# samxuxiang/BrepGen

Measured on AMD Instinct MI355X. Metric: denoising-steps/sec (whole node), DeepCAD face-LDM, batch=512, higher is better.
Workload: dtype bf16

## Files before the change

brepgen_amd/_lib.py:

```python
import ctypes as C
import os

_HERE = os.path.dirname(os.path.abspath(__file__))
LIB_PATH = os.path.join(_HERE, "libbrepgen_hip.so")

BG_F32, BG_F16, BG_BF16 = 0, 1, 2
BG_ACT_NONE, BG_ACT_RELU = 0, 1
BG_SURFPOS, BG_SURFZ, BG_EDGEPOS, BG_EDGEZ = 0, 1, 2, 3
BG_MAX_LAYERS, BG_MAX_EMBEDS = 12, 5
BG_ATTN_BWD_AUTO, BG_ATTN_BWD_GENERAL, BG_ATTN_BWD_SHORT = 0, 1, 2

vp, fp, i64p, u8p = C.c_void_p, C.c_void_p, C.c_void_p, C.c_void_p


class MlpWeights(C.Structure):
    _fields_ = [("w0", vp), ("b0", fp), ("ln_g", fp), ("ln_b", fp), ("w3", vp), ("b3", fp),
                ("k_in", C.c_int), ("n_out", C.c_int), ("n_out_pad", C.c_int), ("w0_dtype", C.c_int),
                ("w0_mfma", fp), ("w0_colsum", fp)]


class LayerWeights(C.Structure):
    _fields_ = [("ln1_g", fp), ("ln1_b", fp), ("ln2_g", fp), ("ln2_b", fp),
                ("w_qkv", vp), ("b_qkv", fp), ("w_o", vp), ("b_o", fp),
                ("w_1", vp), ("b_1", fp), ("w_2", vp), ("b_2", fp),
# ... 120 lines not shown
                               fp, fp, fp, C.c_float, C.c_float, C.c_float, C.c_float, C.c_float, fp,
                               C.c_size_t, vp]),
    "bg_groupnorm_stats": (C.c_int, [fp, fp, C.c_int, C.c_int, C.c_int, C.c_int, C.c_float, vp]),
    "bg_im2col": (C.c_int, [fp, vp] + [C.c_int] * 13 + [fp, fp, fp, C.c_int, C.c_int, fp, vp]),
    "bg_downsample1d_cubic": (C.c_int, [fp, fp, C.c_int, C.c_int, C.c_int, vp]),
    "bg_upsample1d_cubic": (C.c_int, [fp, fp, C.c_int, C.c_int, C.c_int, vp]),
    "bg_small_attn": (C.c_int, [fp, C.c_int, vp, C.c_int, C.c_int, C.c_int, C.c_int, C.c_int, C.c_float, vp]),
    "bg_dedup_surfaces": (C.c_int, [fp, C.c_float, fp, u8p, C.c_int, C.c_int, vp]),
    "bg_dedup_edges": (C.c_int, [fp, u8p, C.c_float, u8p, C.c_int, C.c_int, C.c_int, vp]),
    "bg_profile_begin": (C.c_int, [C.c_int]),
    "bg_profile_end": (C.c_int, [C.POINTER(ProfileRow), C.c_int]),
    "bg_tune_set": (C.c_int, [C.c_int, C.c_int]),
    "bg_allgather": (C.c_int, [vp, vp, C.c_size_t, vp, vp]),
    "bg_slot_packing_applies": (C.c_int, [C.c_int] * 6),
    "bg_gemm_p256_rows": (C.c_int, [C.c_int, C.c_int, C.c_int, C.c_int]),
    "bg_add_noise": (C.c_int, [fp, fp, fp, fp, fp, C.c_int, C.c_size_t, vp]),
    "bg_chamfer_offset_fit": (C.c_int, [fp, fp, vp, C.c_int, C.c_int, C.c_int] + [C.c_double] * 5 + [fp, fp, fp, vp]),
    "bg_philox_randn": (C.c_int, [fp, C.c_longlong, C.c_int, C.c_ulonglong, C.c_uint, C.c_longlong, C.c_int, vp]),
    "bg_masked_mse": (C.c_int, [fp, fp, u8p, C.c_longlong, C.c_int, C.c_int, C.c_int, vp, fp, vp]),
    "bg_chamfer_pairwise": (C.c_int, [fp, C.c_int, C.c_int, fp, C.c_int, C.c_int, fp, vp]),
    "bg_occupancy_counts": (C.c_int, [fp, C.c_int, C.c_int, fp, C.c_int, vp, vp, vp]),
    "bg_mesh_sample": (C.c_int, [fp, vp, C.c_int, C.c_int, C.c_ulonglong, C.c_uint, C.c_longlong, fp, fp, fp, vp, fp, vp]),
    "bg_vae_posterior": (C.c_int, [fp, fp, C.c_longlong, C.c_int, C.c_int, C.c_ulonglong, C.c_uint, C.c_longlong, fp, fp, fp, vp]),
    "bg_cad_filter": (C.c_int, [C.POINTER(CadStore), C.c_int, C.c_int, C.c_float, C.c_double, u8p, vp]),
    "bg_batch_plan": (C.c_int, [C.POINTER(CadStore), vp, C.c_int, C.c_int, C.c_int, C.c_int, C.c_int, C.c_ulonglong, C.c_uint,
                                C.POINTER(BatchDraws), vp, vp, vp, fp, vp]),
    "bg_batch_gather": (C.c_int, [C.POINTER(CadStore), C.c_int, C.c_int, C.c_int, C.c_int, C.c_float, vp, vp, vp, fp,
                                  C.POINTER(BatchOut), vp]),
    "bg_points_rotate_normalize": (C.c_int, [fp, C.c_longlong, C.c_int, C.c_int, C.c_ulonglong, C.c_uint, C.c_longlong, fp, vp, fp, vp]),
    "bg_points_sha256": (C.c_int, [fp, C.c_longlong, C.c_int, C.c_int, u8p, vp]),
# ... 110 lines not shown
```

brepgen_amd/csrc/bg_common.h:

```cpp
#pragma once
#include <hip/hip_runtime.h>
#include <stdint.h>
#include <stddef.h>
#include <type_traits>
#include "../../include/brepgen_hip.h"

namespace bg {

void set_error(const char* fmt, ...);
int launch_status(const char* what);

#define BG_REQUIRE(cond, code, ...)            \
    do {                                       \
        if (!(cond)) {                         \
            ::bg::set_error(__VA_ARGS__);      \
            return (code);                     \
        }                                      \
    } while (0)

inline bool aligned(const void* p, size_t bytes) { return ((uintptr_t)p & (bytes - 1)) == 0; }
template <typename F> inline void with_bools(bool a, bool b, F&& f) {
    if (a && b) f(std::true_type{}, std::true_type{});
    else if (a) f(std::true_type{}, std::false_type{});
    else if (b) f(std::false_type{}, std::true_type{});
// ... 1 lines not shown
}

enum ProfKernel { PK_GEMM_BF16_128 = 0,   PK_GEMM_BF16_64, PK_GEMM_F32, PK_ATTN_BF16, PK_ATTN_F32, PK_LAYERNORM,
                  PK_DDPM_STEP, PK_PNDM_STEP, PK_MISC, PK_EMBED, PK_GEMM_P256, PK_GEMM_SPLIT, PK_GEMM_P256_SPLIT, PK_QKV_ATTN, PK_OUT_TAIL, PK_FFN_FUSED, PK_COUNT };
extern bool g_prof_on;
void prof_pre(hipStream_t s);
void prof_post(int kernel, double flops, double bytes, hipStream_t s);
struct ProfScope {
    int k; double f, b; hipStream_t s;
    ProfScope(int kernel, double flops, double bytes, hipStream_t st) : k(kernel), f(flops), b(bytes), s(st) {
        if (g_prof_on) prof_pre(s);
    }
    ~ProfScope() { if (g_prof_on) prof_post(k, f, b, s); }
};

enum TuneKey { TUNE_GEMM_STAGGER = 8, TUNE_P256_MODE = 10, TUNE_SPLIT_PIPE = 12, TUNE_QKV_ATTN = 13, TUNE_QKV_WALK = 14, TUNE_SMALL_TILES = 15, TUNE_FFN_FUSED = 16, TUNE_DEBUG_PTR_LO = 17, TUNE_DEBUG_PTR_HI = 18, TUNE_VAE_GN1_FUSED = 19, TUNE_ATTN_WALK = 20, TUNE_COUNT = 21 };
extern int g_tune[TUNE_COUNT];

typedef __attribute__((ext_vector_type(8))) __bf16 bf16x8;
typedef __attribute__((ext_vector_type(4))) __bf16 bf16x4;
typedef __attribute__((ext_vector_type(4))) _Float16 half4_t;
typedef __attribute__((ext_vector_type(8))) _Float16 half8_t;
typedef __attribute__((ext_vector_type(16))) float f32x16;
typedef __attribute__((ext_vector_type(4))) float f32x4;
typedef __attribute__((ext_vector_type(8))) float f32x8;

constexpr int WAVE = 64;

__device__ __forceinline__ float wave_sum(float v) {
#pragma unroll
    for (int o = 32; o > 0; o >>= 1) v += __shfl_xor(v, o, 64);
// ... 55 lines not shown
    int gemv_ok = 0;
    const int* m_dev = nullptr;
    const int* row_map = nullptr;
    int map_add = 0, map_add2 = 0, map_out = 0;
    double rows_hint = 0.0;
    double rows_plan = 0.0;
    int cv_C = 0, cv_H = 0, cv_W = 0, cv_kh = 1, cv_kw = 1, cv_up = 0;
    int cv_wo_log2 = 0, cv_ho_log2 = 0, cv_spt_log2 = 0;
    const void* cv_zero = nullptr;
    int hybrid = 0;
    const int* rule_table = nullptr;
    const int* rows256_dev = nullptr;
    int rows256_host = 0;
    int p256_stagger = 0;
    int concurrent = 0;
};

inline GemmArgs linear(const void* a, int lda, const void* w, const float* bias, void* out, int ldc, int M, int N, int N_pad, int K,
                       int out_dtype, int act = BG_ACT_NONE) {
    return GemmArgs{a, lda, w, bias, out, ldc, M, N, N_pad, K, out_dtype, act, nullptr, 0, 1};
}
inline void add_rows(GemmArgs& g, const float* add, int ld, int div) { g.add = add; g.ld_add = ld; g.add_div = add ? div : 1; }
inline void add2_rows(GemmArgs& g, const float* add2, int ld, int div) { g.add2 = add2; g.ld_add2 = ld; g.add2_div = add2 ? div : 1; }
inline void split_out(GemmArgs& g, void* lo, float* stats) { g.out_lo = lo; g.stats_out = stats; }
inline void split_residual_in(GemmArgs& g, const void* hi, const void* lo, int ld) { g.res_hi = hi; g.res_lo = lo; g.ld_res = ld; }
inline void ln_fold_in(GemmArgs& g, const float* stats, const float* colsum) { g.stats_in = stats; g.colsum = colsum; }
inline void map_rows(GemmArgs& g, const int* row_map, bool add, bool add2, bool out) {
    g.row_map = row_map; g.map_add = add; g.map_add2 = add2; g.map_out = out;
}

// ... 17 lines not shown
    if (rem == 0 || rem >= 200) return panels << 8;
    return (R * q) << 8;
}
__host__ __device__ inline int p256_rows(int rows, int nt_n256, bool split = false, bool all_or_nothing = false) {
    const int panels = (rows + 255) >> 8, T = panels * nt_n256;
    if (all_or_nothing) {
        if (split) return p256_split_rows(panels, nt_n256, true);
        return (T >= 300 || (T >= 200 && T <= 256)) ? panels << 8 : 0;
    }
    if (split) {
        return p256_split_rows(panels, nt_n256, false);
    }
    const int R = T >> 8, rem = T - (R << 8);
    if (rem == 0 || rem >= P256_TAIL_MIN) return panels << 8;
    return ((R << 8) / nt_n256) << 8;
}

template <bool F16> __device__ __forceinline__ void unpack4_16(uint2 u, float (&f)[4]) {
    if (F16) {
        union { uint2 u; half4_t h; } c; c.u = u;
        f[0] = (float)c.h[0]; f[1] = (float)c.h[1]; f[2] = (float)c.h[2]; f[3] = (float)c.h[3];
    } else {
        f[0] = __uint_as_float(u.x << 16); f[1] = __uint_as_float(u.x & 0xffff0000u);
        f[2] = __uint_as_float(u.y << 16); f[3] = __uint_as_float(u.y & 0xffff0000u);
    }
}
template <bool F16> __device__ __forceinline__ void split4_16(const float (&v)[4], uint2& hi, uint2& lo) {
    hi = pack4_16(v[0], v[1], v[2], v[3], F16 ? BG_F16 : BG_BF16);
    float h[4];
    unpack4_16<F16>(hi, h);
// ... 37 lines not shown
                 int silu, hipStream_t s, const int* m_dev = nullptr, double rows_hint = 0.0);
int layernorm768_split(const void* hi, const void* lo, const float* g, const float* b, void* y, int y_dtype, int M,
                       float eps, hipStream_t s, const int* m_dev = nullptr, double rows_hint = 0.0);
bool embed_ln_silu_supported(int k);
bool gn1_norm_act_supported(int P, int C);
int gn1_norm_act(const float* x, void* out, int out_dtype, int S, int P, int C, const float* gamma, const float* beta, float eps,
                 int act, const float* add, hipStream_t s);
int embed_ln_silu(const float* x, int lda, int rows, int k, const float* w0p, const float* b0, const float* g,
                  const float* b, void* out, int out_dtype, float eps, hipStream_t s, const int* m_dev = nullptr,
                  const int* src_row = nullptr, double rows_hint = 0.0);
int attention(const void* qkv, const uint8_t* key_pad, void* out, int B, int N, int dtype, hipStream_t s,
              const int* offsets = nullptr, double pairs_hint = 0.0, double rows_hint = 0.0);
bool qkv_attn_eligible(int B, int N, int dtype, const void* stats_in, const void* colsum, const void* bias);
bool qkv_attn_worthwhile(int B, int N);
int qkv_attention(const void* x_hi, const void* w_qkv, const float* bias, const float* colsum, const float* stats_in, void* out,
                  const uint8_t* key_pad, int B, int N, int dtype, float ln_eps, hipStream_t s);

int qkv_attention_paired(const void* x_hi, const void* w_qkv, const float* bias, const float* colsum, const float* stats_in, void* out,
                         void* qkv_dbg, const int* m_dev, const int* slot_desc, int slot_bound, int m_stats, int dtype, float ln_eps,
                         hipStream_t s, double rows_hint, double pairs_hint);
int compact_rows_paired(const uint8_t* mask, int B, int n_mask, int* offsets, int* src_row, int* slot_desc, int* slot_a, int* counts,
                        hipStream_t s, int* rule = nullptr);
int compact_rows(const uint8_t* mask, int B, int n_mask, int rep, int* offsets, int* src_row, hipStream_t s, int* rule = nullptr);
int sincos_embed(const int64_t* t, int n, float* out, hipStream_t s);
int cond_vector(const float* temb, int nt, const float* class_embed, const int64_t* label, float* c, int B,
                hipStream_t s);
int cond_vector_table(const float* table, int table_rows, const int64_t* timesteps, int nt, const float* class_embed,
                      const int64_t* label, float* c, int B, hipStream_t s);
bool ln_silu_out_supported(int n_out, int n_out_pad);
int ln_silu_out(const void* t0, const float* gam, const float* bet, const void* w3, const float* b3, float* out, int n_out, int n_out_pad,
                int M, int dtype, float eps, hipStream_t s, const int* m_dev = nullptr, const int* row_map = nullptr, double rows_hint = 0.0);
// ... 16 lines not shown
```

brepgen_amd/csrc/denoiser.hip:

```cpp
#include "bg_common.h"
#include <mutex>

namespace bg {

__global__ void expand_mask_kernel(const uint8_t* __restrict__ in, uint8_t* __restrict__ out, size_t n, int E) {
    for (size_t i = blockIdx.x * (size_t)blockDim.x + threadIdx.x; i < n; i += (size_t)gridDim.x * blockDim.x)
        out[i] = in[i / E];
}

static inline size_t align_up(size_t v) { return (v + 255) & ~(size_t)255; }

struct Workspace {
    size_t off_x, off_h, off_r, off_small, off_f, off_mask, off_stats, off_rows, off_slots, total;
    int M, F;
    int Mrow;
};

static inline bool slot_packing_applies(int net, int B, int S, int E, int dtype) {
    return net == BG_SURFZ && E == 1 && S <= 64 && dtype != BG_F32 && B <= 8192;
}

static Workspace plan(int net, int B, int S, int E, int dtype) {
    Workspace w{};
    const size_t es = (dtype == BG_F32) ? 4 : 2;
// ... 26 lines not shown
    float* X;
    void* H;
    void* R;
    bool fold = false;
    void* XH = nullptr;
    void* XL = nullptr;
    float* stats = nullptr;
    const int* m_dev = nullptr;
    const int* src_row = nullptr;
    const int* offsets = nullptr;
    const int* rule = nullptr;
    const int* slot_desc = nullptr;
    double rows_hint = 0.0, pairs_hint = 0.0;
    double rows_plan = 0.0;
    int concurrent = 0;
    const bg_denoiser_inputs* in = nullptr;
    int net = 0, B = 0, N = 1, E = 1, M = 0;
    bool varlen = false;
    bool paired = false;
    bool fused_qkv = false;
    const uint8_t* key_pad = nullptr;
    float* cvec = nullptr;
};

static void token_rows(const Ctx& c, GemmArgs& g, bool launch_plan = true) {
    g.m_dev = c.m_dev; g.rows_hint = c.rows_hint;
    if (launch_plan) { g.rule_table = c.rule; g.rows_plan = c.rows_plan; g.concurrent = c.concurrent; }
}

struct Addend { const float* rows = nullptr; int ld = 0; int div = 1; };
enum EmbedOpt : unsigned { TO_STREAM = 1, TOK = 2, GATHER = 4, MAP_ADD = 8, MAP_ADD2 = 16, SCATTER = 32 };

static int embed_mlp(Ctx& c, const bg_mlp_weights& m, const void* x, int lda, int rows, float* out, int ldc, Addend add = {},
                     Addend add2 = {}, unsigned opt = 0) {
    int rc;
    const bool vl = (opt & TOK) && c.m_dev != nullptr;
    if (m.w0_mfma && m.w0_dtype == BG_F32 && embed_ln_silu_supported(m.k_in)) {
        rc = embed_ln_silu(reinterpret_cast<const float*>(x), lda, rows, m.k_in, m.w0_mfma, m.b0, m.ln_g, m.ln_b, c.H,
                           c.dtype, 1e-5f, c.s, vl ? c.m_dev : nullptr, (vl && (opt & GATHER)) ? c.src_row : nullptr, vl ? c.rows_hint : 0.0);
        if (rc) return rc;
    } else {
        BG_REQUIRE(!(vl && (opt & GATHER)), BG_E_ARG, "bg_denoiser_fwd: variable-length execution needs the fused input embeds (w0_mfma)");
// ... 40 lines not shown
    if ((rc = gemm(f1, c.dtype, c.s))) return rc;
    GemmArgs f2 = linear(c.R, 1024, L.w_2, L.b_2, c.X, 768, M, 768, 768, 1024, BG_F32);
    add_rows(f2, c.X, 768, 1);
    token_rows(c, f2);
    return gemm(f2, c.dtype, c.s);
}

static int encoder_layer_folded(const Ctx& c, const bg_layer_weights& L) {
    int rc;
    const int M = c.M;
    if (c.paired) {
        if ((rc = qkv_attention_paired(c.XH, L.w_qkv, L.b_qkv, L.qkv_colsum, c.stats, c.H, nullptr, c.m_dev, c.slot_desc,
                                       c.B < (M + 63) / 64 ? c.B : (M + 63) / 64, M, c.dtype,
                                       1e-5f, c.s, c.rows_hint, c.pairs_hint))) return rc;
    } else if (c.fused_qkv) {
        if ((rc = qkv_attention(c.XH, L.w_qkv, L.b_qkv, L.qkv_colsum, c.stats, c.H, c.key_pad, c.B, c.N, c.dtype, 1e-5f, c.s))) return rc;
    } else {
        GemmArgs qkv = linear(c.XH, 768, L.w_qkv, L.b_qkv, c.R, 2304, M, 2304, 2304, 768, c.dtype);
        ln_fold_in(qkv, c.stats, L.qkv_colsum);
        token_rows(c, qkv);
        if ((rc = gemm(qkv, c.dtype, c.s))) return rc;
        if ((rc = attention(c.R, c.key_pad, c.H, c.B, c.N, c.dtype, c.s, c.offsets, c.pairs_hint, c.rows_hint))) return rc;
    }
    GemmArgs op = linear(c.H, 768, L.w_o, L.b_o, c.XH, 768, M, 768, 768, 768, c.dtype);
    split_out(op, c.XL, c.stats);
    split_residual_in(op, c.XH, c.XL, 768);
    token_rows(c, op);
    if ((rc = gemm(op, c.dtype, c.s))) return rc;
    if (L.w_1f && L.w_2f && g_tune[TUNE_FFN_FUSED] != 1) {
        FfnArgs ff{c.XH, c.XL, c.stats, L.w_1f, L.b_1, L.w1_colsum, L.w_2f, L.b_2, M, M, c.m_dev, 1e-5f};
        BG_REQUIRE(ffn_fused_eligible(ff, c.dtype), BG_E_ARG, "bg_denoiser_fwd: w_1f / w_2f given, but the fused FFN launch does not apply");
// ... 160 lines not shown
                   "bg_denoiser_fwd: fc_out carries the folded final LayerNorm (w0_colsum): needs the 16-bit LayerNorm-fold layers and n_out <= 48");
        GemmArgs g0 = linear(c.XH, 768, mo.w0, mo.b0, c.H, 768, M, 768, 768, 768, c.dtype);
        ln_fold_in(g0, c.stats, mo.w0_colsum);
        token_rows(c, g0);
        if ((rc = gemm(g0, c.dtype, c.s))) return rc;
        return ln_silu_out(c.H, mo.ln_g, mo.ln_b, mo.w3, mo.b3, eps_out, mo.n_out, mo.n_out_pad, M, c.dtype, 1e-5f, c.s, c.m_dev,
                           c.varlen ? c.src_row : nullptr, c.rows_hint);
    }
    if (c.fold) rc = layernorm768_split(c.XH, c.XL, c.w->lnf_g, c.w->lnf_b, c.H, c.dtype, M, 1e-5f, c.s, c.m_dev, c.rows_hint);
    else rc = layernorm768(c.X, c.w->lnf_g, c.w->lnf_b, c.H, c.dtype, M, 1e-5f, 0, c.s, c.m_dev, c.rows_hint);
    if (rc) return rc;
    return embed_mlp(c, mo, c.H, 768, M, eps_out, mo.n_out, {}, {}, TOK | SCATTER);
}

static int run(const bg_denoiser_weights* w, const bg_denoiser_inputs* in, float* eps_out, void* workspace,
               size_t ws_bytes, hipStream_t s, bool concurrent = false) {
    int rc;
    if ((rc = check_args(w, in, eps_out, workspace))) return rc;
    Ctx c;
    c.s = s;
    c.concurrent = concurrent ? 1 : 0;
    if ((rc = bind_workspace(c, w, in, workspace, ws_bytes))) return rc;
    if (c.varlen && (rc = setup_varlen(c, eps_out))) return rc;
    if ((rc = cond_vectors(c))) return rc;
    if ((rc = token_embeds(c))) return rc;
    if ((rc = encoder_layers(c))) return rc;
    return output_tail(c, eps_out);
}

}

namespace bg {
constexpr int MAX_SPLIT = 4;
static inline void split_range(int B, int n, int k, int& lo, int& hi) {
    const int base = B / n, rem = B % n;
    lo = k * base + (k < rem ? k : rem);
    hi = lo + base + (k < rem ? 1 : 0);
}
static size_t plan_total_split(int net, int B, int S, int E, int dtype, int n) {
    size_t t = 0;
    for (int k = 0; k < n; ++k) {
        int lo, hi;
        split_range(B, n, k, lo, hi);
        if (hi > lo) t += align_up(plan(net, hi - lo, S, E, dtype).total);
    }
    return t;
}
struct SplitState {
    hipStream_t aux[MAX_SPLIT - 1];
    hipEvent_t fork, join[MAX_SPLIT - 1];
    bool tried = false, ok = false;
};
constexpr int MAX_SPLIT_DEVICES = 64;
// ... 18 lines not shown
extern "C" int bg_slot_packing_applies(int net, int B, int S, int E, int dtype, int fold) {
    if (net < BG_EDGEPOS) E = 1;
    return (bg::slot_packing_applies(net, B, S, E, dtype) && fold != 0 && bg::g_tune[bg::TUNE_QKV_ATTN] != 1) ? 1 : 0;
}

extern "C" size_t bg_workspace_bytes(int net, int B, int S, int E, int dtype) {
    if (B <= 0 || S <= 0) return 0;
    if (net < BG_EDGEPOS) E = 1;
    if (E <= 0) return 0;
    size_t t = bg::plan(net, B, S, E, dtype).total;
    for (int n = 2; n <= bg::MAX_SPLIT; ++n) {
        const size_t ts = bg::plan_total_split(net, B, S, E, dtype, n);
        t = ts > t ? ts : t;
    }
    return t;
}

extern "C" int bg_denoiser_fwd(const bg_denoiser_weights* w, const bg_denoiser_inputs* in, float* eps_out,
                               void* workspace, size_t workspace_bytes, bg_stream_t stream) {
    using namespace bg;
    BG_REQUIRE(w && in, BG_E_ARG, "bg_denoiser_fwd: null descriptor");
    hipStream_t s = (hipStream_t)stream;
    BG_REQUIRE(in->n_split >= 0, BG_E_ARG, "bg_denoiser_fwd: n_split must be >= 0 (got %d)", in->n_split);
    const int ns = in->n_split > MAX_SPLIT ? MAX_SPLIT : in->n_split;
    if (ns < 2 || in->B < ns) return run(w, in, eps_out, workspace, workspace_bytes, s);

    const int net = w->net;
    BG_REQUIRE(net >= BG_SURFPOS && net <= BG_EDGEZ, BG_E_ARG, "bg_denoiser_fwd: bad net id %d", net);
    BG_REQUIRE(in->B > 0 && in->S > 0 && eps_out && workspace, BG_E_ARG, "bg_denoiser_fwd: null pointer / empty shape");
    const int S = in->S, E = (net >= BG_EDGEPOS) ? in->E : 1;
// ... 20 lines not shown
        sub.n_split = 1;
        sub.x = in->x + (size_t)lo * tok * kInCols[net];
        if (in->surf_pos) sub.surf_pos = in->surf_pos + (size_t)lo * S * 6;
        if (in->surf_z) sub.surf_z = in->surf_z + (size_t)lo * S * 48;
        if (in->edge_pos) sub.edge_pos = in->edge_pos + (size_t)lo * tok * 6;
        if (in->mask) sub.mask = in->mask + (size_t)lo * mask_per_sample;
        if (in->n_timesteps == in->B) { sub.timesteps = in->timesteps + lo; sub.n_timesteps = sub.B; }
        if (in->class_label) sub.class_label = in->class_label + lo;
        if (in->cond_cache) sub.cond_cache = in->cond_cache + (size_t)lo * S * 768;
        sub.rows_hint = in->rows_hint * sub.B / in->B;
        sub.pairs_hint = in->pairs_hint * sub.B / in->B;
        sub.rows_plan[0] = in->rows_plan[k];
        const size_t bytes = align_up(plan(net, sub.B, S, E, w->dtype).total);
        hipStream_t sk = k == 0 ? s : g_split.aux[k - 1];
        if (k > 0 && (he = hipStreamWaitEvent(sk, g_split.fork, 0)) != hipSuccess) { rc = (int)he; break; }
        rc = run(w, &sub, eps_out + (size_t)lo * tok * w->fc_out.n_out, wsp, bytes, sk, true);
        if (rc) break;
        wsp += bytes;
    }
    for (int k = 1; k < ns; ++k) {
        if (hipEventRecord(g_split.join[k - 1], g_split.aux[k - 1]) == hipSuccess)
            (void)hipStreamWaitEvent(s, g_split.join[k - 1], 0);
    }
    return rc;
}

extern "C" size_t bg_embed_mlp_scratch_bytes(int rows, int dtype) {
    if (rows <= 0) return 0;
    const size_t es = (dtype == BG_F32) ? 4 : 2;
    return bg::align_up((size_t)rows * 768 * es) + bg::align_up((size_t)rows * 768 * 4);
}
// ... 45 lines not shown
```

brepgen_amd/csrc/gemm_16bit.hip:

```cpp
#include "gemm16.h"

namespace bg {

template <bool F16, int BM, int BN, int WM, int WN, int STAGES>
__global__ __launch_bounds__(WM * WN * 64) void gemm16_kernel(GemmArgs g) {
    using E = Elem<F16>;
    using T = typename E::T;
    using V8 = typename E::V8;
    using V4 = typename E::V4;
    constexpr int NW = WM * WN;
    constexpr int TM = BM / WM / 32, TN = BN / WN / 32;
    constexpr int STAGE_BYTES = (BM + BN) * 128;
    constexpr int EH = TM > 2 ? 2 : TM;
    constexpr int EPI_BYTES = NW * EH * 32 * (BN / WN) * 4;
    constexpr int LDS_BYTES = (STAGES * STAGE_BYTES > EPI_BYTES) ? STAGES * STAGE_BYTES : EPI_BYTES;
    static_assert(LDS_BYTES <= 160 * 1024, "LDS budget");
    static_assert((BM / 8) % NW == 0 && (BN / 8) % NW == 0, "DMA pieces must divide evenly over the waves");
    __shared__ __attribute__((aligned(16))) unsigned char lds[LDS_BYTES];

    const T* __restrict__ A = reinterpret_cast<const T*>(g.a);
    const T* __restrict__ W = reinterpret_cast<const T*>(g.w);
    const int lane = threadIdx.x & 63;
    const int wave = __builtin_amdgcn_readfirstlane(threadIdx.x >> 6);
    const int wm = wave / WN, wn = wave % WN;
// ... 667 lines not shown
        return BG_E_SHAPE;
    }
    GemmArgs gt = g;
    gt.hybrid = 0;
    if (g_tune[TUNE_P256_MODE] != 2 && p256_eligible(g)) {
        const bool split = g.out_lo != nullptr;
        const int hmode = g.concurrent ? 2 : 1;
        auto p256 = [&](GemmArgs h, double rows) {
            double fl, by;
            gemm_cost(g, rows, fl, by);
            ProfScope prof(split ? PK_GEMM_P256_SPLIT : PK_GEMM_P256, fl, by, s);
            if (split) h.p256_stagger = split_stagger(g);
            return launch_p256<F16>(h, s);
        };
        if (g_tune[TUNE_P256_MODE] == 1) return p256(g, rows_all);
        const bool plan = g.m_dev != nullptr && g.rows_plan > 0;
        const int rows_est = plan ? (int)fmin((double)g.M, g.rows_plan + 0.5)
                                  : ((g.m_dev != nullptr && g.rows_hint > 0) ? (int)fmin((double)g.M, g.rows_hint + 0.5) : g.M);
        const int rows_hi = p256_rows(rows_est, g.N_pad / 256, split, hmode == 2);
        if (plan && rows_hi >= rows_est) return p256(g, rows_all);
        const int ridx = p256_rule_index(g.N_pad / 256, split, hmode == 2);
        const bool can_tail = persistent_ok && (!g.stats_in || g.K == FOLD_PARTS * G_BK) &&
                              (g.m_dev == nullptr || (g.rule_table != nullptr && ridx >= 0));
        if (rows_hi > 0 && can_tail) {
            gt.hybrid = hmode;
            if (g.m_dev) gt.rows256_dev = g.rule_table + ridx;
            else gt.rows256_host = p256_rows(g.M, g.N_pad / 256, split, hmode == 2);
            const double rows_p = fmin((double)p256_rows((int)rows_all, g.N_pad / 256, split, hmode == 2), rows_all);
            rows_tail = rows_all - rows_p;
            const int rc = p256(gt, rows_p);
// ... 70 lines not shown
```

brepgen_amd/csrc/gemm_split.hip:

```cpp
#include "gemm16.h"

namespace bg {

constexpr int SP_STAGE = 32768, SP_RING = 2 * SP_STAGE, SP_PATCH = 4096;
typedef __attribute__((ext_vector_type(4))) unsigned sp_u32x4;

template <bool F16>
__global__ __launch_bounds__(256, 2) void gemm16_split_pipe_kernel(GemmArgs g, int m_panels) {
    using E = Elem<F16>;
    using T = typename E::T;
    using V8 = typename E::V8;
    __shared__ __attribute__((aligned(16))) unsigned char lds[SP_RING + 4 * SP_PATCH];

    const int lane = threadIdx.x & 63;
    const int wave = __builtin_amdgcn_readfirstlane(threadIdx.x >> 6);
    const int wm = wave >> 1, wn = wave & 1;
    const int l31 = lane & 31, hq = lane >> 5, k8 = lane & 7, r8 = lane >> 3;
    const int Mv = g.m_dev ? *g.m_dev : g.M;
    if (g.m_dev) m_panels = (Mv + 127) >> 7;
    const PanelWalk128 walk(g, m_panels, g.N_pad >> 7, blockIdx.x, gridDim.x);
    const int w_local = walk.w_local, cnt = walk.cnt;

    const unsigned char* Ab = reinterpret_cast<const unsigned char*>(g.a);
    const unsigned char* Wb = reinterpret_cast<const unsigned char*>(g.w);
// ... 213 lines not shown
}

bool split_pipe_eligible(const GemmArgs& g) {
    if (!(g.out_lo && g.res_hi && g.res_lo && g.stats_out && g.bias) || g.stats_in || g.add || g.add2 || g.row_map || g.act != BG_ACT_NONE ||
        g.cv_C > 0 || g.out_dtype == BG_F32)
        return false;
    if (g.N != g.N_pad || g.N_pad % 128 != 0 || g.K % (4 * G_BK) != 0 || g.K < 12 * G_BK || g.ldc % 8 != 0 || g.ld_res % 8 != 0)
        return false;
    const long long nt = (long long)((g.M + 127) / 128) * (g.N_pad / 128);
    return nt >= 64 && (size_t)127 * g.lda * 2 + 128 < 0xffffffffull && (size_t)127 * g.K * 2 + 128 < 0xffffffffull;
}

template <bool F16>
int launch_split_pipe(const GemmArgs& g, hipStream_t s) {
    const int m128 = (g.M + 127) / 128, nt = m128 * (g.N_pad / 128);
    const int grid = nt < 512 ? (nt & ~7) : 512;
    hipLaunchKernelGGL((gemm16_split_pipe_kernel<F16>), dim3(grid), dim3(256), 0, s, g, m128);
    return launch_status("gemm16_split_pipe");
}
template int launch_split_pipe<false>(const GemmArgs&, hipStream_t);
template int launch_split_pipe<true>(const GemmArgs&, hipStream_t);

}
```

brepgen_amd/csrc/qkv_attn.hip:

```cpp
#include "gemm16.h"
#include <math.h>

namespace bg {

constexpr int QA_BUF = 57344, QA_AHALF = 16384, QA_WOFF = 32768, QA_RING = 2 * QA_BUF;
constexpr int QA_LDS = 163840;
constexpr int QA_AUX = QA_RING, QA_BIAS = QA_LDS - QA_AUX - 2048, QA_CSUM = QA_BIAS + 1024;
constexpr int QA_QIMG = QA_BUF, QA_KIMG = QA_QIMG + 32768, QA_VIMG = QA_KIMG + 32768;

constexpr int QA_MB = QA_AUX + QA_BIAS - 1024;
static_assert(QA_VIMG + 32768 <= QA_MB && QA_VIMG + 32768 <= QA_AUX + QA_BIAS, "the V image ends below the key bias / bias / column sums");

struct QkvAttnArgs {
    const void* a;
    const void* w;
    const float* bias;
    const float* colsum;
    const float* stats_in;
    void* out;
    void* dbg;
    const uint8_t* key_pad;
    int B, N, M;
    float ln_eps;
    const int* m_dev = nullptr;
// ... 417 lines not shown
           (((size_t)stats_in) & 15) == 0 && (size_t)B * N * BG_D_MODEL * 2 < 0xffffffffull;
}

bool qkv_attn_worthwhile(int B, int N) {
    const int spt = N <= 32 ? 8 : 4;
    const int tiles = (B + spt - 1) / spt * BG_N_HEAD;
    return tiles <= 256 || tiles >= 352;
}

static int qkv_attn_pinned_walk(int tiles, int grid) {
    const int t = g_tune[TUNE_QKV_WALK];
    if (t == 1 || (grid & 7) != 0) return 0;
    return (t == 2 || tiles >= 512) ? 1 : 0;
}

int qkv_attention_launch(const QkvAttnArgs& g, int dtype, hipStream_t s) {
    const int S = g.N <= 32 ? 32 : 64, spt = 256 / S;
    const int tiles = (g.B + spt - 1) / spt * BG_N_HEAD;
    if (tiles <= 0) return 0;
    const double rows = (double)g.B * g.N;
    ProfScope prof(PK_QKV_ATTN, 2.0 * rows * BG_D_MODEL * 3 * BG_D_MODEL + 4.0 * BG_N_HEAD * (double)g.B * g.N * g.N * BG_D_HEAD,
                   rows * (2.0 * BG_D_MODEL * 2 + FOLD_PARTS * 8.0) + 2.0 * 3 * BG_D_MODEL * BG_D_MODEL + 2 * 4.0 * 3 * BG_D_MODEL, s);
    const int grid = tiles < 256 ? tiles : 256;
    const bool f16 = dtype == BG_F16;
    QkvAttnArgs ge = g;
    ge.pin = qkv_attn_pinned_walk(tiles, grid);
#define QA_LAUNCH(F, SS, MK, D) hipLaunchKernelGGL((qkv_attn_kernel<F, SS, MK, D>), dim3(grid), dim3(512), 0, s, ge)
#define QA_PICK(MK, D)                                                                                     \
    do {                                                                                                   \
        if (S == 64) { if (f16) QA_LAUNCH(true, 64, MK, D); else QA_LAUNCH(false, 64, MK, D); }           \
        else { if (f16) QA_LAUNCH(true, 32, MK, D); else QA_LAUNCH(false, 32, MK, D); }                   \
    } while (0)
    if (g.dbg) {
        if (g.key_pad) QA_PICK(true, true); else QA_PICK(false, true);
    } else {
        if (g.key_pad) QA_PICK(true, false); else QA_PICK(false, false);
    }
#undef QA_PICK
// ... 14 lines not shown
    const double pairs = pairs_hint > 0 ? pairs_hint : 64.0 * rows;
    ProfScope prof(PK_QKV_ATTN, 2.0 * rows * BG_D_MODEL * 3 * BG_D_MODEL + 4.0 * BG_N_HEAD * pairs * BG_D_HEAD,
                   rows * (2.0 * BG_D_MODEL * 2 + FOLD_PARTS * 8.0) + 2.0 * 3 * BG_D_MODEL * BG_D_MODEL + 2 * 4.0 * 3 * BG_D_MODEL, s);
    const int grid = tiles < 256 ? tiles : 256;
    if (dtype == BG_F16) {
        if (qkv_dbg) hipLaunchKernelGGL((qkv_attn_kernel<true, 64, false, true, true>), dim3(grid), dim3(512), 0, s, g);
        else hipLaunchKernelGGL((qkv_attn_kernel<true, 64, false, false, true>), dim3(grid), dim3(512), 0, s, g);
    } else {
        if (qkv_dbg) hipLaunchKernelGGL((qkv_attn_kernel<false, 64, false, true, true>), dim3(grid), dim3(512), 0, s, g);
        else hipLaunchKernelGGL((qkv_attn_kernel<false, 64, false, false, true>), dim3(grid), dim3(512), 0, s, g);
    }
    return launch_status("qkv_attn_paired");
}

int qkv_attention(const void* x_hi, const void* w_qkv, const float* bias, const float* colsum, const float* stats_in, void* out,
                  const uint8_t* key_pad, int B, int N, int dtype, float ln_eps, hipStream_t s) {
    const QkvAttnArgs g{x_hi, w_qkv, bias, colsum, stats_in, out, nullptr, key_pad, B, N, B * N, ln_eps};
    return qkv_attention_launch(g, dtype, s);
}

}

extern "C" int bg_qkv_attn_fwd(const void* x_hi, const void* w_qkv, const float* bias, const float* colsum, const float* stats_in,
                               const uint8_t* key_pad, void* out, void* qkv_dbg, int B, int N, int dtype, float ln_eps,
                               bg_stream_t stream) {
    BG_REQUIRE(x_hi && w_qkv && out && B >= 0 && N >= 0, BG_E_ARG, "bg_qkv_attn_fwd: null pointer or negative size");
    BG_REQUIRE(bg::qkv_attn_eligible(B, N, dtype, stats_in, colsum, bias), BG_E_SHAPE,
               "bg_qkv_attn_fwd: needs 16-bit operands, an even N in [2, 64], LayerNorm-fold statistics / column sums / bias (16-byte aligned)");
    BG_REQUIRE(((uintptr_t)x_hi & 15) == 0 && ((uintptr_t)w_qkv & 15) == 0 && ((uintptr_t)out & 15) == 0 &&
               ((uintptr_t)bias & 15) == 0 && ((uintptr_t)colsum & 15) == 0, BG_E_ALIGN, "bg_qkv_attn_fwd: 16-byte alignment");
    bg::QkvAttnArgs g{x_hi, w_qkv, bias, colsum, stats_in, out, qkv_dbg, key_pad, B, N, B * N, ln_eps};
    return bg::qkv_attention_launch(g, dtype, (hipStream_t)stream);
}
// ... 15 lines not shown
```

brepgen_amd/csrc/runtime.hip:

```cpp
#include "bg_common.h"
#include <stdarg.h>
#include <stdio.h>

namespace bg {

static thread_local char g_err[512] = "";

void set_error(const char* fmt, ...) {
    va_list ap;
    va_start(ap, fmt);
    vsnprintf(g_err, sizeof(g_err), fmt, ap);
    va_end(ap);
}

int launch_status(const char* what) {
    const hipError_t e = hipGetLastError();
    if (e == hipSuccess) return 0;
    set_error("%s: launch failed: %s", what, hipGetErrorString(e));
    return (int)e;
}

int g_tune[TUNE_COUNT] = {0};

bool g_prof_on = false;
// ... 61 lines not shown
        if (agg[k].launches > 0 && rows) rows[n++] = agg[k];
    return n;
}

extern "C" int bg_tune_set(int key, int value) {
    BG_REQUIRE(key >= 0 && key < bg::TUNE_COUNT, BG_E_ARG, "bg_tune_set: unknown key %d", key);
    bg::g_tune[key] = value;
    return 0;
}

extern "C" int bg_gemm_p256_rows(int rows, int n_cols, int split_residual, int concurrent) {
    BG_REQUIRE(rows >= 0 && n_cols > 0 && (n_cols & 255) == 0, BG_E_ARG, "bg_gemm_p256_rows: rows >= 0 and n_cols a positive multiple of 256 expected");
    return bg::p256_rows(rows, n_cols >> 8, split_residual != 0, concurrent != 0);
}

extern "C" int bg_abi_version(void) { return BG_ABI_VERSION; }
extern "C" const char* bg_last_error(void) { return bg::g_err; }
```

brepgen_amd/network.py:

```python
import ctypes as C

import torch
import torch.nn as nn

from . import _lib
from ._lib import (BG_BF16, BG_EDGEPOS, BG_EDGEZ, BG_F16, BG_F32, BG_SURFPOS, BG_SURFZ, DenoiserInputs,
                   DenoiserWeights, check, ptr, stream)

D, H, DFF, NLAYER = 768, 12, 1024, 12


class _Embedder(nn.Module):
    def __init__(self, vocab, dim):
        super().__init__()
        self.embed = nn.Embedding(vocab, dim)
        nn.init.kaiming_normal_(self.embed.weight, mode="fan_in")


class _AttnParams(nn.Module):
    def __init__(self):
        super().__init__()
        self.in_proj_weight = nn.Parameter(torch.empty(3 * D, D))
        self.in_proj_bias = nn.Parameter(torch.zeros(3 * D))
        self.out_proj = nn.Linear(D, D)
# ... 282 lines not shown
        w, _keep = self._pack(dt)
        dev = x.device
        t = timesteps.reshape(-1).to(device=dev, dtype=torch.int64).contiguous()
        if t.numel() not in (1, B):
            raise ValueError("timesteps must hold 1 or batch-size entries")
        mk = None
        if mask is not None:
            mk = mask.contiguous()
            mk = mk.view(torch.uint8) if mk.dtype == torch.bool else mk.to(torch.uint8)
        inp = DenoiserInputs()
        inp.B, inp.S, inp.E, inp.n_timesteps = B, S, E, t.numel()
        inp.x, inp.surf_pos, inp.surf_z, inp.edge_pos = ptr(x), ptr(surf_pos), ptr(surf_z), ptr(edge_pos)
        inp.mask, inp.timesteps, inp.class_label = ptr(mk), ptr(t), ptr(class_label)
        inp.cond_cache, inp.cond_cache_valid = None, 0
        inp.varlen = int(bool(self.varlen) and mk is not None and self.NET != BG_SURFPOS)
        ns = self.n_split
        if ns == "auto":
            ns = 2 if (B >= 2 and B * S * E >= 16384) else 1
        inp.n_split = int(ns)
        (inp.rows_hint, inp.pairs_hint), plan = (0.0, 0.0), ()
        if inp.varlen:
            fold_on = int(dt != torch.float32 and bool(self.fold_layernorm))
            paired = lambda group_b: bool(_lib.load().bg_slot_packing_applies(self.NET, group_b, S, E, w.dtype, fold_on))
            (inp.rows_hint, inp.pairs_hint), plan = self._row_hints(mask, S, E, B, ns, paired)
        for k in range(4):
            inp.rows_plan[k] = plan[k] if k < len(plan) else 0.0
        use_cache = (self.cache_conditioning and surf_pos is not None and not self.training
                     and not torch.cuda.is_current_stream_capturing())
        if use_cache:
            conds = [c for c in (surf_pos, surf_z) if c is not None]
            vers = [c._version for c in conds]
            hit = (self._cond is not None and self._cond["meta"] == (dt, B, S) and
                   len(self._cond["src"]) == len(conds) and
                   all(a is b for a, b in zip(self._cond["src"], conds)) and self._cond["ver"] == vers)
            if not hit:
                self._cond = {"meta": (dt, B, S), "src": conds, "ver": vers, "valid": False,
                              "buf": torch.empty(B * S, D, device=dev, dtype=torch.float32)}
            inp.cond_cache = ptr(self._cond["buf"])
            inp.cond_cache_valid = int(self._cond["valid"])
# ... 93 lines not shown
```

include/brepgen_hip.h:

```cpp
#ifndef BREPGEN_HIP_H
#define BREPGEN_HIP_H

#include <stddef.h>
#include <stdint.h>

#ifdef __cplusplus
extern "C" {
#endif

#define BG_ABI_VERSION 7

typedef void* bg_stream_t;

enum bg_dtype { BG_F32 = 0, BG_F16 = 1, BG_BF16 = 2 };
enum bg_act { BG_ACT_NONE = 0, BG_ACT_RELU = 1 };
enum bg_net { BG_SURFPOS = 0, BG_SURFZ = 1, BG_EDGEPOS = 2, BG_EDGEZ = 3 };
enum bg_err { BG_E_ARG = -1, BG_E_SHAPE = -2, BG_E_WORKSPACE = -3, BG_E_DTYPE = -4, BG_E_ALIGN = -5 };

#define BG_D_MODEL 768
#define BG_N_HEAD 12
#define BG_D_HEAD 64
#define BG_D_FF 1024
#define BG_MAX_LAYERS 12
#define BG_MAX_EMBEDS 5
// ... 180 lines not shown
    const float* surf_z;
    const float* edge_pos;
    const uint8_t* mask;
    const int64_t* timesteps;
    const int64_t* class_label;
    float* cond_cache;
    int cond_cache_valid;
    int varlen;
    double rows_hint, pairs_hint;
    int n_split;
    int _pad2;
    double rows_plan[4];
} bg_denoiser_inputs;

int bg_slot_packing_applies(int net, int B, int S, int E, int dtype, int fold);

size_t bg_workspace_bytes(int net, int B, int S, int E, int dtype);

int bg_denoiser_fwd(const bg_denoiser_weights* w, const bg_denoiser_inputs* in, float* eps_out,
                    void* workspace, size_t workspace_bytes, bg_stream_t stream);

size_t bg_embed_mlp_scratch_bytes(int rows, int dtype);
int bg_embed_mlp_fwd(const bg_mlp_weights* m, int dtype, const void* x, int lda, int rows, float* out, int ldc,
                     const float* add, int ld_add, int add_div, void* scratch, size_t scratch_bytes, bg_stream_t stream);
size_t bg_encoder_layer_scratch_bytes(int B, int N, int dtype);
int bg_encoder_layer_fwd(const bg_layer_weights* L, int dtype, float* x, const uint8_t* key_pad, int B, int N,
                         void* scratch, size_t scratch_bytes, bg_stream_t stream);


int bg_cfg_ddpm_step(const float* eps_c, const float* eps_u, float guidance_w, const float* x,
// ... 58 lines not shown
    const char* kernel;
    int launches;
    double total_ms;
    double flops;
    double bytes;
} bg_profile_row;
int bg_profile_begin(int max_launches);
int bg_profile_end(bg_profile_row* rows, int max_rows);

int bg_allgather(const void* send, void* recv, size_t bytes_per_rank, void* nccl_comm, bg_stream_t stream);

int bg_tune_set(int key, int value);

int bg_gemm_p256_rows(int rows, int n_cols, int split_residual, int concurrent);

int bg_add_noise(const float* x0, const float* noise, const float* sqrt_alpha_prod,
                 const float* sqrt_one_minus_alpha_prod, float* out, int B, size_t per_sample,
                 bg_stream_t stream);

int bg_philox_randn(float* out, long long n_samples, int per_sample, unsigned long long seed, unsigned draw_id,
                    long long first_sample, int raw_bits, bg_stream_t stream);

int bg_chamfer_offset_fit(const float* surf, const float* edge_pts, const int* edge_off, int F, int P, int iters, double lr,
                          double beta1, double beta2, double weight_decay, double eps, float* offsets_out, float* surf_out,
                          float* loss_out, bg_stream_t stream);

int bg_masked_mse(const float* pred, const float* target, const uint8_t* row_mask, long long rows, int ld, int col0,
                  int ncols, double* scratch, float* out3, bg_stream_t stream);


// ... 100 lines not shown
```

Baseline: 370.9.

## Size kernel grids for sibling split streams and move split decision to C

When the denoiser batch is split across concurrent streams, the number of groups is now passed down so the GEMM p256 rule, the split-pipe GEMM grid and the fused QKV-attention grid can size themselves to share the device with the sibling stream. The auto split threshold moves into a C helper and, for varlen inputs, is re-evaluated from the per-group row plan, falling back to one group when groups would be too small. The intent is to cut oversubscription and tail effects when two streams compete for compute units. The risk is under-filling the GPU if the sibling stream is not actually running at the same time.

```diff
diff --git a/brepgen_amd/_lib.py b/brepgen_amd/_lib.py
--- a/brepgen_amd/_lib.py
+++ b/brepgen_amd/_lib.py
@@ -158,6 +158,9 @@
     "bg_allgather": (C.c_int, [vp, vp, C.c_size_t, vp, vp]),
     "bg_slot_packing_applies": (C.c_int, [C.c_int] * 6),
     "bg_gemm_p256_rows": (C.c_int, [C.c_int, C.c_int, C.c_int, C.c_int]),
+    "bg_gemm_p256_rows_groups": (C.c_int, [C.c_int, C.c_int, C.c_int, C.c_int]),
+    "bg_qkv_attn_grid": (C.c_int, [C.c_int, C.c_int, C.c_int]),
+    "bg_denoiser_n_split": (C.c_int, [C.c_int] * 5 + [C.c_double]),
     "bg_add_noise": (C.c_int, [fp, fp, fp, fp, fp, C.c_int, C.c_size_t, vp]),
     "bg_chamfer_offset_fit": (C.c_int, [fp, fp, vp, C.c_int, C.c_int, C.c_int] + [C.c_double] * 5 + [fp, fp, fp, vp]),
     "bg_philox_randn": (C.c_int, [fp, C.c_longlong, C.c_int, C.c_ulonglong, C.c_uint, C.c_longlong, C.c_int, vp]),
diff --git a/brepgen_amd/csrc/bg_common.h b/brepgen_amd/csrc/bg_common.h
--- a/brepgen_amd/csrc/bg_common.h
+++ b/brepgen_amd/csrc/bg_common.h
@@ -39,7 +39,7 @@
     ~ProfScope() { if (g_prof_on) prof_post(k, f, b, s); }
 };
 
-enum TuneKey { TUNE_GEMM_STAGGER = 8, TUNE_P256_MODE = 10, TUNE_SPLIT_PIPE = 12, TUNE_QKV_ATTN = 13, TUNE_QKV_WALK = 14, TUNE_SMALL_TILES = 15, TUNE_FFN_FUSED = 16, TUNE_DEBUG_PTR_LO = 17, TUNE_DEBUG_PTR_HI = 18, TUNE_VAE_GN1_FUSED = 19, TUNE_ATTN_WALK = 20, TUNE_COUNT = 21 };
+enum TuneKey { TUNE_GEMM_STAGGER = 8, TUNE_P256_MODE = 10, TUNE_SPLIT_PIPE = 12, TUNE_QKV_ATTN = 13, TUNE_QKV_WALK = 14, TUNE_SMALL_TILES = 15, TUNE_FFN_FUSED = 16, TUNE_DEBUG_PTR_LO = 17, TUNE_DEBUG_PTR_HI = 18, TUNE_VAE_GN1_FUSED = 19, TUNE_ATTN_WALK = 20, TUNE_SIBLING = 21, TUNE_COUNT = 22 };
 extern int g_tune[TUNE_COUNT];
 
 typedef __attribute__((ext_vector_type(8))) __bf16 bf16x8;
@@ -125,6 +125,7 @@
     int rows256_host = 0;
     int p256_stagger = 0;
     int concurrent = 0;
+    int groups = 0;
 };
 
 inline GemmArgs linear(const void* a, int lda, const void* w, const float* bias, void* out, int ldc, int M, int N, int N_pad, int K,
@@ -172,6 +173,33 @@
     const int R = T >> 8, rem = T - (R << 8);
     if (rem == 0 || rem >= P256_TAIL_MIN) return panels << 8;
     return ((R << 8) / nt_n256) << 8;
+}
+
+__host__ __device__ inline int p256_rows_groups(int rows, int nt_n256, bool split, int groups) {
+    if (groups < 2) return p256_rows(rows, nt_n256, split, false);
+    const int own = p256_rows(rows, nt_n256, split, true);
+    if (own > 0 || split) return own;
+    const int panels = (rows + 255) >> 8;
+    const long long T = (long long)panels * nt_n256 * groups;
+    return (T >= 200 && T <= 256) ? panels << 8 : 0;
+}
+__host__ __device__ inline int split_pipe_grid(int nt, int groups, bool full = false) {
+    const int own = nt < 512 ? (nt & ~7) : 512;
+    if (groups < 2 || (nt >= 512 && !full)) return own;
+    const int share = (512 / groups) & ~7;
+    return own < share ? own : share;
+}
+__host__ __device__ inline int qkv_attn_grid(int tiles, int groups, bool full = false) {
+    const int own = tiles < 256 ? tiles : 256;
+    if (groups < 2 || tiles < 256 || (tiles >= 512 && !full)) return own;
+    return (256 / groups) & ~7;
+}
+enum SiblingPlan { SIBLING_RULE_256 = 1, SIBLING_GRID_SPLIT = 2, SIBLING_GRID_SPLIT_FULL = 4, SIBLING_FORCED = 8, SIBLING_GRID_QKV = 16,
+                   SIBLING_GRID_QKV_FULL = 32 };
+constexpr int SIBLING_PLAN_SHIPPED = SIBLING_RULE_256 | SIBLING_GRID_QKV;
+inline int sibling_plan() {
+    const int t = g_tune[TUNE_SIBLING];
+    return t > 0 ? (t - 1) & 63 : SIBLING_PLAN_SHIPPED;
 }
 
 template <bool F16> __device__ __forceinline__ void unpack4_16(uint2 u, float (&f)[4]) {
@@ -239,7 +267,7 @@
 bool qkv_attn_eligible(int B, int N, int dtype, const void* stats_in, const void* colsum, const void* bias);
 bool qkv_attn_worthwhile(int B, int N);
 int qkv_attention(const void* x_hi, const void* w_qkv, const float* bias, const float* colsum, const float* stats_in, void* out,
-                  const uint8_t* key_pad, int B, int N, int dtype, float ln_eps, hipStream_t s);
+                  const uint8_t* key_pad, int B, int N, int dtype, float ln_eps, hipStream_t s, int groups = 0);
 
 int qkv_attention_paired(const void* x_hi, const void* w_qkv, const float* bias, const float* colsum, const float* stats_in, void* out,
                          void* qkv_dbg, const int* m_dev, const int* slot_desc, int slot_bound, int m_stats, int dtype, float ln_eps,
diff --git a/brepgen_amd/csrc/denoiser.hip b/brepgen_amd/csrc/denoiser.hip
--- a/brepgen_amd/csrc/denoiser.hip
+++ b/brepgen_amd/csrc/denoiser.hip
@@ -64,6 +64,7 @@
     double rows_hint = 0.0, pairs_hint = 0.0;
     double rows_plan = 0.0;
     int concurrent = 0;
+    int groups = 0;
     const bg_denoiser_inputs* in = nullptr;
     int net = 0, B = 0, N = 1, E = 1, M = 0;
     bool varlen = false;
@@ -75,7 +76,7 @@
 
 static void token_rows(const Ctx& c, GemmArgs& g, bool launch_plan = true) {
     g.m_dev = c.m_dev; g.rows_hint = c.rows_hint;
-    if (launch_plan) { g.rule_table = c.rule; g.rows_plan = c.rows_plan; g.concurrent = c.concurrent; }
+    if (launch_plan) { g.rule_table = c.rule; g.rows_plan = c.rows_plan; g.concurrent = c.concurrent; g.groups = c.groups; }
 }
 
 struct Addend { const float* rows = nullptr; int ld = 0; int div = 1; };
@@ -146,7 +147,7 @@
                                        c.B < (M + 63) / 64 ? c.B : (M + 63) / 64, M, c.dtype,
                                        1e-5f, c.s, c.rows_hint, c.pairs_hint))) return rc;
     } else if (c.fused_qkv) {
-        if ((rc = qkv_attention(c.XH, L.w_qkv, L.b_qkv, L.qkv_colsum, c.stats, c.H, c.key_pad, c.B, c.N, c.dtype, 1e-5f, c.s))) return rc;
+        if ((rc = qkv_attention(c.XH, L.w_qkv, L.b_qkv, L.qkv_colsum, c.stats, c.H, c.key_pad, c.B, c.N, c.dtype, 1e-5f, c.s, c.groups))) return rc;
     } else {
         GemmArgs qkv = linear(c.XH, 768, L.w_qkv, L.b_qkv, c.R, 2304, M, 2304, 2304, 768, c.dtype);
         ln_fold_in(qkv, c.stats, L.qkv_colsum);
@@ -337,12 +338,13 @@
 }
 
 static int run(const bg_denoiser_weights* w, const bg_denoiser_inputs* in, float* eps_out, void* workspace,
-               size_t ws_bytes, hipStream_t s, bool concurrent = false) {
+               size_t ws_bytes, hipStream_t s, bool concurrent = false, int groups = 0) {
     int rc;
     if ((rc = check_args(w, in, eps_out, workspace))) return rc;
     Ctx c;
     c.s = s;
     c.concurrent = concurrent ? 1 : 0;
+    c.groups = concurrent ? groups : 0;
     if ((rc = bind_workspace(c, w, in, workspace, ws_bytes))) return rc;
     if (c.varlen && (rc = setup_varlen(c, eps_out))) return rc;
     if ((rc = cond_vectors(c))) return rc;
@@ -360,6 +362,7 @@
     lo = k * base + (k < rem ? k : rem);
     hi = lo + base + (k < rem ? 1 : 0);
 }
+constexpr int SPLIT_MIN_GROUP_ROWS = 8192;
 static size_t plan_total_split(int net, int B, int S, int E, int dtype, int n) {
     size_t t = 0;
     for (int k = 0; k < n; ++k) {
@@ -408,6 +411,15 @@
         t = ts > t ? ts : t;
     }
     return t;
+}
+
+extern "C" int bg_denoiser_n_split(int net, int B, int S, int E, int dtype, double rows_per_group) {
+    BG_REQUIRE(net >= BG_SURFPOS && net <= BG_EDGEZ, BG_E_ARG, "bg_denoiser_n_split: bad net id %d", net);
+    BG_REQUIRE(dtype == BG_F32 || dtype == BG_BF16 || dtype == BG_F16, BG_E_DTYPE, "bg_denoiser_n_split: dtype %d", dtype);
+    if (net < BG_EDGEPOS) E = 1;
+    if (B < 2 || S <= 0 || E <= 0) return 1;
+    const double rows = rows_per_group > 0 ? rows_per_group : 0.5 * (double)B * S * E;
+    return rows >= (double)bg::SPLIT_MIN_GROUP_ROWS ? 2 : 1;
 }
 
 extern "C" int bg_denoiser_fwd(const bg_denoiser_weights* w, const bg_denoiser_inputs* in, float* eps_out,
@@ -458,7 +470,7 @@
         const size_t bytes = align_up(plan(net, sub.B, S, E, w->dtype).total);
         hipStream_t sk = k == 0 ? s : g_split.aux[k - 1];
         if (k > 0 && (he = hipStreamWaitEvent(sk, g_split.fork, 0)) != hipSuccess) { rc = (int)he; break; }
-        rc = run(w, &sub, eps_out + (size_t)lo * tok * w->fc_out.n_out, wsp, bytes, sk, true);
+        rc = run(w, &sub, eps_out + (size_t)lo * tok * w->fc_out.n_out, wsp, bytes, sk, true, ns);
         if (rc) break;
         wsp += bytes;
     }
diff --git a/brepgen_amd/csrc/gemm_16bit.hip b/brepgen_amd/csrc/gemm_16bit.hip
--- a/brepgen_amd/csrc/gemm_16bit.hip
+++ b/brepgen_amd/csrc/gemm_16bit.hip
@@ -705,6 +705,10 @@
             return launch_p256<F16>(h, s);
         };
         if (g_tune[TUNE_P256_MODE] == 1) return p256(g, rows_all);
+        const int sib = g.m_dev == nullptr && g.groups >= 2 ? sibling_plan() : 0;
+        if (((sib & SIBLING_FORCED) && !split) || ((sib & SIBLING_RULE_256) && p256_rows(g.M, g.N_pad / 256, split, true) == 0 &&
+                          p256_rows_groups(g.M, g.N_pad / 256, split, g.groups) >= g.M))
+            return p256(g, rows_all);
         const bool plan = g.m_dev != nullptr && g.rows_plan > 0;
         const int rows_est = plan ? (int)fmin((double)g.M, g.rows_plan + 0.5)
                                   : ((g.m_dev != nullptr && g.rows_hint > 0) ? (int)fmin((double)g.M, g.rows_hint + 0.5) : g.M);
diff --git a/brepgen_amd/csrc/gemm_split.hip b/brepgen_amd/csrc/gemm_split.hip
--- a/brepgen_amd/csrc/gemm_split.hip
+++ b/brepgen_amd/csrc/gemm_split.hip
@@ -251,7 +251,9 @@
 template <bool F16>
 int launch_split_pipe(const GemmArgs& g, hipStream_t s) {
     const int m128 = (g.M + 127) / 128, nt = m128 * (g.N_pad / 128);
-    const int grid = nt < 512 ? (nt & ~7) : 512;
+    const int sib = sibling_plan();
+    int grid = split_pipe_grid(nt, (sib & SIBLING_GRID_SPLIT) ? g.groups : 0, (sib & SIBLING_GRID_SPLIT_FULL) != 0);
+    if ((sib & SIBLING_FORCED) && g.groups >= 2 && grid >= 16) grid = (grid / 2) & ~7;
     hipLaunchKernelGGL((gemm16_split_pipe_kernel<F16>), dim3(grid), dim3(256), 0, s, g, m128);
     return launch_status("gemm16_split_pipe");
 }
diff --git a/brepgen_amd/csrc/qkv_attn.hip b/brepgen_amd/csrc/qkv_attn.hip
--- a/brepgen_amd/csrc/qkv_attn.hip
+++ b/brepgen_amd/csrc/qkv_attn.hip
@@ -455,14 +455,16 @@
     return (t == 2 || tiles >= 512) ? 1 : 0;
 }
 
-int qkv_attention_launch(const QkvAttnArgs& g, int dtype, hipStream_t s) {
+int qkv_attention_launch(const QkvAttnArgs& g, int dtype, hipStream_t s, int groups = 0) {
     const int S = g.N <= 32 ? 32 : 64, spt = 256 / S;
     const int tiles = (g.B + spt - 1) / spt * BG_N_HEAD;
     if (tiles <= 0) return 0;
     const double rows = (double)g.B * g.N;
     ProfScope prof(PK_QKV_ATTN, 2.0 * rows * BG_D_MODEL * 3 * BG_D_MODEL + 4.0 * BG_N_HEAD * (double)g.B * g.N * g.N * BG_D_HEAD,
                    rows * (2.0 * BG_D_MODEL * 2 + FOLD_PARTS * 8.0) + 2.0 * 3 * BG_D_MODEL * BG_D_MODEL + 2 * 4.0 * 3 * BG_D_MODEL, s);
-    const int grid = tiles < 256 ? tiles : 256;
+    const int sib = groups >= 2 ? sibling_plan() : 0;
+    int grid = qkv_attn_grid(tiles, (sib & SIBLING_GRID_QKV) ? groups : 0, (sib & SIBLING_GRID_QKV_FULL) != 0);
+    if ((sib & SIBLING_FORCED) && grid >= 16) grid = (grid / 2) & ~7;
     const bool f16 = dtype == BG_F16;
     QkvAttnArgs ge = g;
     ge.pin = qkv_attn_pinned_walk(tiles, grid);
@@ -507,9 +509,9 @@
 }
 
 int qkv_attention(const void* x_hi, const void* w_qkv, const float* bias, const float* colsum, const float* stats_in, void* out,
-                  const uint8_t* key_pad, int B, int N, int dtype, float ln_eps, hipStream_t s) {
+                  const uint8_t* key_pad, int B, int N, int dtype, float ln_eps, hipStream_t s, int groups) {
     const QkvAttnArgs g{x_hi, w_qkv, bias, colsum, stats_in, out, nullptr, key_pad, B, N, B * N, ln_eps};
-    return qkv_attention_launch(g, dtype, s);
+    return qkv_attention_launch(g, dtype, s, groups);
 }
 
 }
diff --git a/brepgen_amd/csrc/runtime.hip b/brepgen_amd/csrc/runtime.hip
--- a/brepgen_amd/csrc/runtime.hip
+++ b/brepgen_amd/csrc/runtime.hip
@@ -99,5 +99,17 @@
     return bg::p256_rows(rows, n_cols >> 8, split_residual != 0, concurrent != 0);
 }
 
+extern "C" int bg_gemm_p256_rows_groups(int rows, int n_cols, int split_residual, int groups) {
+    BG_REQUIRE(rows >= 0 && n_cols > 0 && (n_cols & 255) == 0 && groups >= 0, BG_E_ARG,
+               "bg_gemm_p256_rows_groups: rows >= 0, n_cols a positive multiple of 256 and groups >= 0 expected");
+    return bg::p256_rows_groups(rows, n_cols >> 8, split_residual != 0, groups);
+}
+
+extern "C" int bg_qkv_attn_grid(int B, int N, int groups) {
+    BG_REQUIRE(B > 0 && B <= (1 << 24) && N >= 2 && N <= 64 && groups >= 0, BG_E_ARG, "bg_qkv_attn_grid: 0 < B <= 2^24, 2 <= N <= 64 and groups >= 0 expected");
+    const int spt = N <= 32 ? 8 : 4;
+    return bg::qkv_attn_grid((B + spt - 1) / spt * BG_N_HEAD, groups);
+}
+
 extern "C" int bg_abi_version(void) { return BG_ABI_VERSION; }
 extern "C" const char* bg_last_error(void) { return bg::g_err; }
diff --git a/brepgen_amd/network.py b/brepgen_amd/network.py
--- a/brepgen_amd/network.py
+++ b/brepgen_amd/network.py
@@ -320,15 +320,19 @@
         inp.mask, inp.timesteps, inp.class_label = ptr(mk), ptr(t), ptr(class_label)
         inp.cond_cache, inp.cond_cache_valid = None, 0
         inp.varlen = int(bool(self.varlen) and mk is not None and self.NET != BG_SURFPOS)
-        ns = self.n_split
-        if ns == "auto":
-            ns = 2 if (B >= 2 and B * S * E >= 16384) else 1
-        inp.n_split = int(ns)
+        ns, auto = self.n_split, self.n_split == "auto"
+        if auto:
+            ns = _lib.load().bg_denoiser_n_split(self.NET, B, S, E, w.dtype, 0.0)
         (inp.rows_hint, inp.pairs_hint), plan = (0.0, 0.0), ()
         if inp.varlen:
             fold_on = int(dt != torch.float32 and bool(self.fold_layernorm))
             paired = lambda group_b: bool(_lib.load().bg_slot_packing_applies(self.NET, group_b, S, E, w.dtype, fold_on))
             (inp.rows_hint, inp.pairs_hint), plan = self._row_hints(mask, S, E, B, ns, paired)
+            if auto and ns > 1 and plan:
+                ns = _lib.load().bg_denoiser_n_split(self.NET, B, S, E, w.dtype, max(plan))
+                if ns == 1:
+                    (inp.rows_hint, inp.pairs_hint), plan = self._row_hints(mask, S, E, B, ns, paired)
+        inp.n_split = int(ns)
         for k in range(4):
             inp.rows_plan[k] = plan[k] if k < len(plan) else 0.0
         use_cache = (self.cache_conditioning and surf_pos is not None and not self.training
diff --git a/include/brepgen_hip.h b/include/brepgen_hip.h
--- a/include/brepgen_hip.h
+++ b/include/brepgen_hip.h
@@ -218,6 +218,8 @@
 } bg_denoiser_inputs;
 
 int bg_slot_packing_applies(int net, int B, int S, int E, int dtype, int fold);
+
+int bg_denoiser_n_split(int net, int B, int S, int E, int dtype, double rows_per_group);
 
 size_t bg_workspace_bytes(int net, int B, int S, int E, int dtype);
 
@@ -306,6 +308,9 @@
 
 int bg_gemm_p256_rows(int rows, int n_cols, int split_residual, int concurrent);
 
+int bg_gemm_p256_rows_groups(int rows, int n_cols, int split_residual, int groups);
+int bg_qkv_attn_grid(int B, int N, int groups);
+
 int bg_add_noise(const float* x0, const float* noise, const float* sqrt_alpha_prod,
                  const float* sqrt_one_minus_alpha_prod, float* out, int B, size_t per_sample,
                  bg_stream_t stream);
```

After: 370.6, median of 2. No clear change (-0.1%).
